# DeepOptimalControl/DeepPicardIteration

Hardware: AMD Instinct MI355X
Metric: SDE-path labels/sec (100-d, 50 Euler steps) per GPU; rel-L2 vs ref (higher is better)
Workload: dtype f32

## Files before the change

deeppicarditeration_amd/_lib.py:

```python
import ctypes
import os
from pathlib import Path

_HERE = Path(__file__).resolve().parent
LIB_PATH = Path(os.environ.get("DPI_HIP_LIB", _HERE / "libdpi_hip.so"))

DPI_ABI_VERSION = 8
DPI_LAUNCH_TIMERS = 256
DPI_OK, DPI_ERR_ARG, DPI_ERR_UNSUPPORTED, DPI_ERR_HIP, DPI_ERR_WORKSPACE = 0, -1, -2, -3, -4
DPI_TAG_T, DPI_TAG_X0, DPI_TAG_X, DPI_TAG_TERM, DPI_TAG_S, DPI_TAG_INT, DPI_TAG_SDGD, DPI_TAG_HTERM, DPI_TAG_HINT = range(1, 10)
DPI_EQ_CHA, DPI_EQ_OU, DPI_EQ_GBM = 1, 2, 3
DPI_ACT_ELU, DPI_ACT_TANH = 1, 2
DPI_HEAD_VALUE, DPI_HEAD_VALUE_GRADIENT, DPI_HEAD_GRADIENT = 0, 1, 2
DPI_TERMINAL, DPI_INTEGRAL, DPI_BOTH = 1, 2, 3
DPI_PREPARED = 4
DPI_PATH_BLOCK = 64
DPI_PATHS_PER_CALL_MAX = 1024 * DPI_PATH_BLOCK
DPI_GEMM_F32, DPI_GEMM_F16X3, DPI_GEMM_AUTO = 0, 1, 2
DPI_STATUS_NONFINITE = 1
DPI_STATUS_HANDOFF = 2
DPI_STATUS_SLOTS = 64
DPI_FAMILY_SPECIALISED, DPI_FAMILY_GENERAL = 0, 1

c_int, c_double, c_float, c_size_t, c_void_p, c_uint32, c_uint64 = (
    ctypes.c_int, ctypes.c_double, ctypes.c_float, ctypes.c_size_t, ctypes.c_void_p, ctypes.c_uint32, ctypes.c_uint64)
P = ctypes.POINTER

SIGNATURES = {
    "dpi_abi_version": (c_int, []),
    "dpi_last_error": (c_int, [ctypes.c_char_p, c_size_t]),
    "dpi_problem_create_cha": (c_int, [c_int, c_double, c_double, c_double, P(c_void_p)]),
    "dpi_problem_create_ou": (c_int, [c_int, c_double, c_double, c_double, c_double, c_double, c_int,
                                      P(c_double), P(c_double), P(c_double), P(c_void_p)]),
    "dpi_problem_create_gbm": (c_int, [c_int, c_double, c_double, c_int, P(c_double), P(c_double), P(c_void_p)]),
    "dpi_problem_set_hessian_approximation": (c_int, [c_void_p, c_int]),
    "dpi_problem_set_estimate_delta_t": (c_int, [c_void_p, c_double]),
    "dpi_problem_destroy": (c_int, [c_void_p]),
    "dpi_net_create_zero": (c_int, [P(c_void_p)]),
    "dpi_net_create_mlp": (c_int, [c_int, c_int, P(c_int), c_int, P(c_float), c_size_t, P(c_void_p)]),
    "dpi_net_create_mlp_head": (c_int, [c_int, c_int, P(c_int), c_int, c_int, P(c_float), c_size_t, P(c_void_p)]),
    "dpi_net_create_mlp_terminal": (c_int, [c_int, c_int, P(c_int), c_int, c_int, c_double, P(c_float), c_size_t,
                                            P(c_void_p)]),
    "dpi_net_create_pisgrad": (c_int, [c_int, c_int, P(c_int), c_double, P(c_float), c_size_t, P(c_void_p)]),
    "dpi_net_destroy": (c_int, [c_void_p]),
    "dpi_pair_family": (c_int, [c_void_p, c_void_p, c_int, P(c_int)]),
    "dpi_general_slots": (c_int, [c_void_p, P(c_int)]),
    "dpi_set_gemm_precision": (c_int, [c_int]),
    "dpi_net_set_precision": (c_int, [c_void_p, c_int]),
    "dpi_net_status": (c_int, [c_void_p, c_int, c_void_p, P(c_int)]),
# ... 100 lines not shown
```

deeppicarditeration_amd/csrc/dpi_device.h:

```cpp
#pragma once
#include <hip/hip_runtime.h>
#include <stdint.h>

#include <cmath>
#include <cstdio>
#include <cstring>
#include <cstdlib>
#include <type_traits>
#include <algorithm>
#include <string>
#include <vector>

#include "../../include/dpi.h"
#include "dpi_eq.h"
#include "dpi_rng.h"

namespace dpi {

typedef float floatx4 __attribute__((ext_vector_type(4)));

constexpr int P = DPI_PATH_BLOCK;
constexpr int NTH = 256;
constexpr int SS = P + 4;
constexpr int WST = 136;
#ifndef DPI_NOISE_UNROLL_FO
#define DPI_NOISE_UNROLL_FO 4
#endif
#ifndef DPI_NOISE_UNROLL_GBM
#define DPI_NOISE_UNROLL_GBM 8
#endif
#ifndef DPI_GBM_WAGPR
#define DPI_GBM_WAGPR 1
#endif
#ifndef DPI_WV_UNIFORM_GBM
#define DPI_WV_UNIFORM_GBM 0
#endif
#ifndef DPI_NOISE_UNROLL_HESS
#define DPI_NOISE_UNROLL_HESS 4
#endif
#ifndef DPI_NOISE_TABLE_FO
#define DPI_NOISE_TABLE_FO 1
#endif
constexpr int NXP_MAX = 128;
constexpr int NXW_MAX = 256;
constexpr int HBS = NXW_MAX;
constexpr int HMAX = 128;

struct NetDev {
  int kind;
  int H, L, nxp;
  int act;
  const float* W1x;
  const float* w1t;
  const float* b1;
  const float* c1;
  const float* W1xT;
  const float* W[4];
  const float* WT[4];
  const float* b[4];
  const float* wout;
  float bout;
  int nxp32;
  const uint32_t* W1xS;
  const uint32_t* W1xTS;
  const uint32_t* WS[4];
  const uint32_t* WTS[4];
  const uint32_t* WU[4];
  float wus[4];
  float hsa[4], hsc[4], hzs[4], hbs[4];
};

__device__ __forceinline__ floatx4 mfma4(float a, float b, floatx4 c) {
  return __builtin_amdgcn_mfma_f32_16x16x4f32(a, b, c, 0, 0, 0);
}
// ... 1512 lines not shown
    for (int g = 0; g < 16; ++g) a += udp[g][tid];
    hb[(size_t)i * HBS + c0 + tid] = c0 + tid < nx ? a : 0.f;
  }
  if (NXW > NXP_MAX) __syncthreads();
  }
  if (tid == 0) fb[i] = Cb;
}

}
#include "dpi_general.h"
namespace dpi {

struct PathArgs {
  const float* tx;
  const float* gx;
  const float* fb;
  const float* bx;
  const float* hb;
  float* partial;
  int n, nbp, m_begin, m_end, K, flags;
  uint32_t k0, k1, c3t, c3s, c3i, c3q, point_base;
  int order;
  int split;
  float* hpart;
  uint32_t c3h1, c3h2;
  float td_dt;
  int* tickets;
  float* rd_moments;
  float* rd_y;
  int* rd_status;
  float rd_invM, rd_bound;
  int rd_add_g;
  const float* noise;
};

struct FusedBase {
  int nbase;
  float* rec;
  unsigned long long* ready;
  uint32_t ready_seq;
  SampleSpec smp;
};

__device__ __forceinline__ unsigned long long ready_word(uint32_t seq) {
  return ((unsigned long long)seq << 32) | (unsigned long long)(~seq);
}
__device__ __forceinline__ void base_publish(const FusedBase& fb, int i) {
  asm volatile("s_waitcnt vmcnt(0)" ::: "memory");
  __syncthreads();
  if (threadIdx.x == 0) {
    __builtin_amdgcn_fence(__ATOMIC_RELEASE, "agent");
    asm volatile("s_waitcnt vmcnt(0)" ::: "memory");
    __hip_atomic_store(fb.ready + i, ready_word(fb.ready_seq), __ATOMIC_RELAXED, __HIP_MEMORY_SCOPE_AGENT);
  }
}
constexpr int BASE_SPIN_MAX = 1 << 20;
__device__ __forceinline__ int& base_ok() {
  __shared__ int ok;
  return ok;
}
__device__ __forceinline__ void base_poll(const FusedBase& fb, const PathArgs& a, int i) {
  if (threadIdx.x == 0) {
    const unsigned long long want = ready_word(fb.ready_seq);
    int it = 0;
    while (__hip_atomic_load(fb.ready + i, __ATOMIC_RELAXED, __HIP_MEMORY_SCOPE_AGENT) != want &&
           ++it < BASE_SPIN_MAX)
      __builtin_amdgcn_s_sleep(8);
// ... 485 lines not shown
      }
    }
  };
  auto integral_rollout = [&]() {
#pragma unroll
    for (int c = 0; c < NBW; ++c) {
      const int j = (3 - wv) + 4 * c;
      if (j < nb) {
        float s0 = 0.f, s1 = 0.f, s2 = 0.f, s3 = 0.f;
        if (INTG && !PRE) {
          noise_sums<NOISE_UNROLL, NOISE_FORM>(a.K, nb, j, m, ig, a.c3i, a.k0, a.k1, s0, s1, s2, s3, ntab);
        }
        float sv[4] = {s0 * BM_SCALE, s1 * BM_SCALE, s2 * BM_SCALE, s3 * BM_SCALE};
        if (INTG && PRE) {
          const float* np = a.noise + ((size_t)(i * a.nbp + blk) * 2 + 1) * (4 * nb) * P + lane;
#pragma unroll
          for (int q = 0; q < 4; ++q) sv[q] = np[(4 * j + q) * P];
        }
#pragma unroll
        for (int q = 0; q < 4; ++q) {
          const int d = 4 * j + q;
          sh.S[d * SS + lane] = d < nx ? sv[q] : 0.f;
          if constexpr (GBM) {
            if (d < nx) {
#pragma unroll
              for (int c = 0; c < NSG; ++c)
                if (c < e.nodes) fst[c] = fmaf(e.gw[c * F + 1 + d], sv[q], fst[c]);
            }
          }
        }
      }
    }
  };
  auto terminal_finish = [&]() -> float {
#pragma unroll
    for (int c = 0; c < NSG; ++c) sh.gst[(wv * P + lane) * NSG + c] = gst[c];
    if constexpr (GBM) {
#pragma unroll
      for (int c = 0; c < NSG; ++c) sh.fst[(wv * P + lane) * NSG + c] = fst[c];
    }
    __syncthreads();
    float gT = 0.f;
    if (TERM) {
#pragma unroll
      for (int c = 0; c < NSG; ++c)
        gst[c] = ((sh.gst[(0 * P + lane) * NSG + c] + sh.gst[(1 * P + lane) * NSG + c]) +
                  sh.gst[(2 * P + lane) * NSG + c]) + sh.gst[(3 * P + lane) * NSG + c];
      gT = Eq<KIND>::gfin(e, gst);
    }
    return TERM ? gT - g_x : 0.f;
  };

  auto integrand = [&]() {
    if constexpr (!GBM) {
      float u = 0.f, gs = 0.f, gA = 0.f, gB = 0.f;
      if (!ZERO && INTG) {
        if constexpr (GEN)
          mlp_tile_gen<KIND, H, ACT, NET, TERMA>(e, net, sh, stash, u, gs, gA, gB);
        else if constexpr (SPLIT)
          mlp_tile_split<KIND, H, L, ACT>(e, net, sh, u, gs, gA, gB);
        else
          mlp_tile<KIND, H, L, ACT>(e, net, sh, nxp / 16, u, gs, gA, gB, nullptr, 0, P);
      }
      const int pp = 16 * wv + (lane & 15);
      if ((lane >> 4) == 0) sh.bsh[pp] = INTG ? tmt * (Eq<KIND>::ffv(e, u, gs, gA, gB) - f_b) : 0.f;
    } else {
      const int jj = lane & 15, qq = lane >> 4, pp = 16 * wv + jj;
      float s1 = 0.f, s2 = 0.f;
      if constexpr (!ZERO) {
        if (INTG) {
          if constexpr (SPLIT)
            mlp_hdiag_split<H, L, ACT>(e, net, sh, nxp / 16, s1, s2);
          else
            mlp_hdiag<H, L, ACT>(e, net, sh, nxp / 16, s1, s2);
        }
      }
      const float vv = (float)(e.sdgd_v > 0 ? e.sdgd_v : nx);
      const float c1 = 0.5f * (1.0f - e.alpha) * (float)nx / vv, c2 = 0.25f * (float)nx / vv;
      float arg[NSG], sn[NSG];
      const float spp = sh.tau[pp], cpp = sh.cmul[pp];
#pragma unroll
      for (int c = 0; c < NSG; ++c) {
        arg[c] = 0.f;
        if (c < e.nodes) {
          const float ws = ((sh.fst[(0 * P + pp) * NSG + c] + sh.fst[(1 * P + pp) * NSG + c]) +
                            sh.fst[(2 * P + pp) * NSG + c]) + sh.fst[(3 * P + pp) * NSG + c];
          arg[c] = fmaf(e.gw[c * F], spp, fmaf(cpp, ws, sh.wx[c]));
        }
        sn[c] = __sinf(arg[c]);
      }
      const float ah = qsum(Eq<KIND>::abs_hess_partial(e, sn, qq, 4));
      float b1 = 0.f, b2 = 0.f;
      for (int d = qq; d < nx; d += 4) {
        const float c = (float)sh.cnt[d * P + pp], h = sh.hb[d];
        b1 = fmaf(c, h, b1);
        b2 = fmaf(c, fabsf(h), b2);
      }
      b1 = qsum(b1);
      b2 = qsum(b2);
      const float f = c1 * s1 + c2 * s2 + Eq<KIND>::exact_scalar_terms(e, arg) - 0.25f * ah;
      const float fbp = f_b + c1 * b1 + c2 * b2;
      if (qq == 0) {
        sh.bsh[pp] = INTG ? tmt * (f - fbp) : 0.f;
        sh.fbp[pp] = fbp;
      }
    }
  };

  bool tlast = false;
  if constexpr (TD) {
    tlast = false;
  } else if constexpr (GEN) {
    tlast = true;
  } else if constexpr (SPLIT && !GBM) {
    tlast = true;
  } else if constexpr (!GBM) {
    if (a.order == 1) tlast = (__builtin_amdgcn_s_getreg((3 << 11) | (16 << 6) | 4) & 1) != 0;
    else if (a.order == 2) tlast = (bid & 1) != 0;
    else if (a.order == 3) tlast = ((bid >> 8) & 1) != 0;
    else if (a.order == 4) tlast = true;
  }
  [[maybe_unused]] auto terminal_value_td = [&]() -> float {
#pragma unroll
    for (int c = 0; c < NBW; ++c) {
      const int j = wv + 4 * c;
      if (j < nb)
#pragma unroll
        for (int q = 0; q < 4; ++q) {
          const int d = 4 * j + q;
          sh.S[d * SS + lane] = d < nx ? ST[c][q] : 0.f;
        }
    }
    if (wv == 0) {
      sh.tau[lane] = t + a.td_dt;
      sh.cmul[lane] = cT;
    }
    __syncthreads();
    float u = 0.f;
    if constexpr (!ZERO) {
      if constexpr (GBM) {
        u = mlp_value_res<H, L, ACT>(net, sh, nxp / 16);
      } else if constexpr (!GEN) {
        float gs, gA, gB;
        if constexpr (SPLIT)
          mlp_tile_split<KIND, H, L, ACT>(e, net, sh, u, gs, gA, gB);
        else
          mlp_tile<KIND, H, L, ACT>(e, net, sh, nxp / 16, u, gs, gA, gB, nullptr, 0, P);
      }
    }
    const int pp = 16 * wv + (lane & 15);
    if ((lane >> 4) == 0) sh.bsh[pp] = u;
    __syncthreads();
    const float uT = sh.bsh[lane];
    if (wv == 0) {
      sh.tau[lane] = s;
      sh.cmul[lane] = cI;
    }
    return uT;
  };
  auto base_poll_ = [&]() {
    if constexpr (FBC) base_poll(fb, a, i);
  };
  auto base_load = [&]() {
    if constexpr (FBC) {
      const bool ok = base_ok() != 0;
      const float* r = fb.rec + (size_t)i * BREC;
      g_x = uniform_f(ok ? rec_load(r) : __builtin_nanf(""));
      f_b = uniform_f(ok ? rec_load(r + 1) : __builtin_nanf(""));
      if (!ZERO) {
        for (int h = tid; h < H; h += NTH) sh.vec[h] = r[32 + h];
        __syncthreads();
      }
    }
  };
  float ap;
  if constexpr (TD) {
    terminal_rollout();
    float uT = 0.f;
    if (td_u && TERM) uT = terminal_value_td();
    integral_rollout();
    ap = terminal_finish();
    if (td_u) ap = TERM ? uT - g_x : 0.f;
    integrand();
    __syncthreads();
  } else if (!tlast) {
    terminal_rollout();
    integral_rollout();
    if constexpr (FBC) {
      base_poll_();
      __syncthreads();
      base_load();
    }
    ap = terminal_finish();
    integrand();
    __syncthreads();
  } else {
    integral_rollout();
    base_poll_();
    __syncthreads();
    base_load();
    integrand();
    terminal_rollout();
    ap = terminal_finish();
  }

  constexpr bool MASK_SCALAR = KIND == DPI_EQ_OU && H == 128 && L == 4 && SPLIT && !TD && NXW == NXP_MAX;
  const bool live = MASK_SCALAR ? lane < a.m_end - a.m_begin - P * blk : m < (uint32_t)a.m_end;
  ap = live ? ap : 0.f;
  const float bp = sh.bsh[lane];
  float* out = a.partial + ((size_t)i * a.nbp + blk) * slab_row(F);
  const float aY = ap * yT, bY = live ? bp * yI : 0.f;
  if constexpr (NXW == NXP_MAX) {
    float col[64];
  #pragma unroll
    for (int c = 0; c < 64; ++c) col[c] = 0.f;
  #pragma unroll
    for (int c = 0; c < 7; ++c) {
// ... 56 lines not shown
          for (int q = 0; q < 4; ++q) {
            const int d = 4 * j + q;
            const float v = d < nx ? fmaf(aY, ST[g0 + c < NBW ? g0 + c : 0][q], bY * sh.S[d * SS + lane]) : 0.f;
            col[8 * c + 2 * q] = v;
            col[8 * c + 2 * q + 1] = v * v;
          }
        }
      }
      if (g0 == 0 && wv == 0) {
        float fbt;
        if constexpr (GBM)
          fbt = sh.fbp[lane];
        else
          fbt = f_b + Eq<KIND>::ffc(e);
        const float c0 = ap + (live ? bp : 0.f) + (INTG ? (live ? fbt : 0.f) * tmt : 0.f);
        col[56] = c0;
        col[57] = c0 * c0;
      }
      const float tot = column_sums64(col);
      const int c = lane >> 3, q = (lane >> 1) & 3, sq = lane & 1;
      const int j = wv + 4 * (g0 + c), d = 4 * j + q;
      if (lane < 56) {
        if (g0 + c < NBW && j < nb && d < nx) out[sq * F + 1 + d] = tot;
      } else if (g0 == 0 && wv == 0 && lane < 58) {
        out[sq * F] = tot;
      }
    }
  }
  if constexpr (HESS) {
    hess_block<KIND, H, L, ZERO, SPLIT, ACT>(e, net, a, sh, i, blk, ig, m, s, smt, tmt, g_x, nxp);
  } else {
    if (a.tickets) fused_reduce(a, i, F, FB ? fb.rec : nullptr);
  }
}

template <int KIND, int H, int L, bool ZERO, bool SPLIT, bool HESS = false, bool TD = false, int ACT = DPI_ACT_ELU,
          int NXW = NXP_MAX>
__global__ __launch_bounds__(256, (k_paths_wgs<KIND, H, L, SPLIT, TD, NXW>())) void k_paths(EqDev e, NetDev net, PathArgs a) {
  paths_body<KIND, H, L, ZERO, SPLIT, HESS, TD, ACT, false, NXW>(e, net, a, FusedBase{});
}
template <int KIND, int H, int L, bool ZERO, bool SPLIT, int ACT = DPI_ACT_ELU>
__global__ __launch_bounds__(256, (k_paths_wgs<KIND, H, L, SPLIT, false>())) void k_paths_fb(EqDev e, NetDev net,
                                                                                            PathArgs a, FusedBase fb) {
  paths_body<KIND, H, L, ZERO, SPLIT, false, false, ACT, true>(e, net, a, fb);
}
template <int KIND, int HCAP, int ACT>
__global__ __launch_bounds__(256, (gen_wgs(HCAP))) void k_paths_gen(EqDev e, NetGen net, PathArgs a, floatx4* stash,
                                                                  unsigned block0) {
  floatx4* const slot = stash + (size_t)blockIdx.x * (gen_slot_floats(net.L, net.ht) / 4);
  paths_body<KIND, HCAP, GEN_LMAX, false, false, false, false, ACT, false, NXP_MAX, NetGen>(e, net, a, FusedBase{},
                                                                                             block0 + blockIdx.x, slot);
}
template <int KIND, int HCAP, int ACT>
__global__ __launch_bounds__(256, (gen_wgs(HCAP))) void k_paths_head(EqDev e, NetGenHead net, PathArgs a) {
  paths_body<KIND, HCAP, GEN_LMAX, false, false, false, false, ACT, false, NXP_MAX, NetGenHead>(e, net, a, FusedBase{},
                                                                                                 blockIdx.x, nullptr);
}
template <int KIND, int HCAP, int ACT>
__global__ __launch_bounds__(256, (gen_wgs(HCAP))) void k_paths_term(EqDev e, NetGen net, PathArgs a, floatx4* stash,
                                                                   unsigned block0) {
  floatx4* const slot = stash + (size_t)blockIdx.x * (gen_slot_floats(net.L, net.ht) / 4);
  paths_body<KIND, HCAP, GEN_LMAX, false, false, false, false, ACT, false, NXP_MAX, NetGen, true>(
      e, net, a, FusedBase{}, block0 + blockIdx.x, slot);
}
template <int KIND, int HCAP, int ACT>
__global__ __launch_bounds__(256, (gen_wgs(HCAP))) void k_paths_head_term(EqDev e, NetGenHead net, PathArgs a) {
// ... 6 lines not shown
```

deeppicarditeration_amd/csrc/dpi_kernels.hip:

```cpp
#include <hip/hip_runtime.h>
#include <stdint.h>

#include <climits>
#include <cmath>
#include <cstdio>
#include <cstring>
#include <cstdlib>
#include <type_traits>
#include <algorithm>
#include <atomic>
#include <mutex>
#include <string>
#include <unordered_map>
#include <vector>

#include "../../include/dpi.h"
#include "dpi_eq.h"
#include "dpi_rng.h"

#include "dpi_dispatch.h"
#include "dpi_pisnet.h"

namespace dpi {

// ... 1258 lines not shown
  L.INP = x3 ? (PIS_CH + pd.nx + 31) & ~31 : r4(PIS_CH + pd.nx);
  o += L.INP;
  L.H0 = o;
  o += PIS_CH;
  L.H1 = o;
  o += PIS_CH;
  for (int l = 0; l < 4; ++l) {
    L.A[l] = o;
    o += l < pd.L ? rw(pd.h[l]) : 0;
  }
  L.NO = o;
  o += rw(pd.nx);
  L.D0 = o;
  o += rw(hmax);
  L.D1 = o;
  o += rw(hmax);
  L.GX = o;
  o += rw(pd.nx);
  L.SS = o;
  o += rw(pd.nx);
  L.ST = o;
  o += rw(pd.nx);
  L.SC = o;
  o += rw(PIS_GST + PIS_PARTS * NSG);
  L.stride = o;
  return L;
}
static int pis_chunk_wg() {
  static const int x = env_int("DPI_PIS_CHUNK", 4096);
  return x >= 1 ? x : 4096;
}

struct WsLayout {
  size_t gx, fb, bx, hb, tk, rec, ready, rows, partial, rq, noise, nq, stash, total;
  int rows_cap;
};
static size_t al256(size_t x) { return (x + 255) & ~size_t(255); }
static bool gbm_noise_prep(dpi_problem p, dpi_net net) {
  static const bool on = env_int("DPI_GBM_PREP", 1) != 0;
  return on && p && net && net->d.kind == 1 && p->e.kind == DPI_EQ_GBM;
}
static WsLayout ws_layout(dpi_net net, int n, int M, int F, bool noise = false) {
  WsLayout w;
  const int H = (net && net->d.kind == 1) ? std::max(net->spec ? net->d.H : 0, net->gen ? net->g.H : 0) : 0;
  const size_t nbp = (size_t)(M + P - 1) / P;
  w.gx = 0;
  w.fb = al256((size_t)n * 4);
  w.bx = w.fb + al256((size_t)n * 4);
  w.hb = w.bx + al256((size_t)n * H * 4);
  w.tk = w.hb + al256((size_t)n * HBS * 4);
  w.rec = w.tk + al256((size_t)n * 4);
  w.ready = w.rec + al256((size_t)n * BREC * 4);
  w.rows = w.ready + al256((size_t)n * 8);
  w.rows_cap = 0;
  size_t rows_bytes = 0;
  if (net && net->d.kind == 2) {
    w.rows_cap = (int)std::min((size_t)n * nbp * P, (size_t)pis_chunk_wg() * P) + n;
    const int stride = std::max(pis_rows_layout(net->pis, false).stride, pis_rows_layout(net->pis, true).stride);
    rows_bytes = al256((size_t)w.rows_cap * stride * 4);
  }
  w.partial = w.rows + rows_bytes;
  w.rq = w.partial + al256((size_t)n * nbp * slab_row(F) * 4);
  w.noise = w.rq + ((net && net->d.kind == 2) ? 256 + (size_t)PIS_CLAIM_SLOTS * 4 : 0);
  const size_t nb4 = (size_t)((F - 1 + 3) / 4) * 4;
  w.nq = w.noise + (noise ? al256((size_t)n * nbp * 2 * nb4 * P * 4) : 0);
  w.total = w.nq + (noise ? 256 + (size_t)PIS_CLAIM_SLOTS * 4 : 0);
  w.stash = w.total;
  if (net && net->d.kind == 1 && net->gen && !net->head) {
    w.stash = al256(w.total);
    w.total = w.stash + al256((size_t)gen_slots(net->g.H) * gen_slot_floats(net->g.L, net->g.ht) * 4);
  }
  return w;
}

static int g_gemm_mode = -1;
static int gemm_mode() {
  if (g_gemm_mode < 0) {
    const char* e = std::getenv("DPI_GEMM");
    g_gemm_mode = !e ? DPI_GEMM_AUTO : std::strcmp(e, "f16x3") == 0 ? DPI_GEMM_F16X3
                                   : std::strcmp(e, "f32") == 0   ? DPI_GEMM_F32
                                                                  : DPI_GEMM_AUTO;
  }
  return g_gemm_mode;
}
static int net_mode(dpi_net net) { return (net && net->precision >= 0) ? net->precision : gemm_mode(); }
static bool mlp_split(dpi_net net) { return net_mode(net) != DPI_GEMM_F32; }
static bool pis_x3(dpi_net net) { return net_mode(net) != DPI_GEMM_F32; }
static int* net_status(dpi_net net) {
  return (net && net->finite && net->status) ? net->status + (size_t)net->slot * STATUS_STRIDE : nullptr;
}

extern "C" int dpi_set_gemm_precision(int mode) {
  if (mode != DPI_GEMM_F32 && mode != DPI_GEMM_F16X3 && mode != DPI_GEMM_AUTO)
    return fail(DPI_ERR_ARG, "gemm precision: 0 = fp32, 1 = fp16-split, 2 = auto");
  g_gemm_mode = mode;
  return 0;
}

template <class F>
static void with_epi(int epi, F f) {
  if (epi == EPI_BIAS)
    f(std::integral_constant<int, EPI_BIAS>{});
  else if (epi == EPI_BIAS_ELU)
// ... 142 lines not shown
  gemm(EPI_BIAS_ELU, R, C, 2 * C, rows + L.E, ld, pd.te0, 2 * C, rows + L.T1, ld, pd.te0b, nullptr, 0, st);
  gemm(EPI_BIAS, R, C, C, rows + L.T1, ld, pd.te2, C, rows + L.IN, ld, pd.te2b, nullptr, 0, st);
  int hs = L.H0, ho = L.H1;
  gemm(EPI_BIAS_ELU, R, C, 2 * C, rows + L.E, ld, pd.sn0, 2 * C, rows + hs, ld, pd.sn0b, nullptr, 0, st);
  for (int j = 0; j < pd.nsm; ++j) {
    gemm(EPI_BIAS_ELU, R, C, C, rows + hs, ld, pd.sn[j], C, rows + ho, ld, pd.snb[j], nullptr, 0, st);
    std::swap(hs, ho);
  }
  int in = C + nx;
  const float* a = rows + L.IN;
  for (int l = 0; l < pd.L; ++l) {
    gemm(EPI_BIAS_ELU, R, pd.h[l], in, a, ld, pd.nn[l], in, rows + L.A[l], ld, pd.nnb[l], nullptr, 0, st);
    a = rows + L.A[l];
    in = pd.h[l];
  }
  gemm(EPI_BIAS, R, nx, in, a, ld, pd.nn[pd.L], in, rows + L.NO, ld, pd.nnb[pd.L], nullptr, 0, st);
  L.H0 = hs;
  if (!vjp) return L;
  int dcur = L.D0, dnext = L.D1;
  gemm(EPI_DELU, R, pd.h[pd.L - 1], nx, rows + L.IN + PIS_IN_OFF, ld, pd.nnT[pd.L], nx, rows + dcur, ld, nullptr,
       rows + L.A[pd.L - 1], ld, st);
  for (int l = pd.L - 1; l >= 1; --l) {
    gemm(EPI_DELU, R, pd.h[l - 1], pd.h[l], rows + dcur, ld, pd.nnT[l], pd.h[l], rows + dnext, ld, nullptr,
         rows + L.A[l - 1], ld, st);
    std::swap(dcur, dnext);
  }
  gemm(EPI_BIAS, R, nx, pd.h[0], rows + dcur, ld, pd.nnT[0], pd.h[0], rows + L.GX, ld, nullptr, nullptr, 0, st);
  L.H0 = hs;
  return L;
}

extern "C" size_t dpi_workspace_bytes(dpi_problem p, dpi_net net, int n, int M) {
  if (!p || n < 0 || M < 0) return 0;
  return ws_layout(net, n, M, 1 + p->e.nx).total;
}
extern "C" size_t dpi_workspace_bytes_prepared(dpi_problem p, dpi_net net, int n, int M) {
  if (!p || n < 0 || M < 0) return 0;
  return ws_layout(net, n, M, 1 + p->e.nx, gbm_noise_prep(p, net)).total;
}

static SampleSpec sample_spec(dpi_problem p, uint64_t seed, uint32_t epoch, uint32_t point_base, float eps,
                              int t_factors, float* tx) {
  SampleSpec s;
  s.tx = tx;
  s.k0 = (uint32_t)seed;
  s.k1 = (uint32_t)(seed >> 32);
  s.c3t = DPI_TAG_T | (epoch << 8);
  s.c3x0 = DPI_TAG_X0 | (epoch << 8);
  s.c3x = DPI_TAG_X | (epoch << 8);
  s.point_base = point_base;
  s.eps = eps;
  s.alpha_init_sqrt = p->alpha_init_sqrt;
  s.t_factors = t_factors;
  return s;
}

extern "C" int dpi_sample_points(dpi_problem p, int n, uint64_t seed, uint32_t epoch, uint32_t point_base, float eps,
                      float* tx, void* stream) {
  return dpi_sample_points_t(p, n, seed, epoch, point_base, eps, 0, tx, stream);
}

extern "C" int dpi_sample_points_t(dpi_problem p, int n, uint64_t seed, uint32_t epoch, uint32_t point_base, float eps,
                                   int t_factors, float* tx, void* stream) {
  if (!p || (!tx && n) || n < 0 || epoch > 0xFFFFFFu || t_factors < 0 || t_factors > 4096)
    return fail(DPI_ERR_ARG, "sample_points: bad arguments (t_factors in [0, 4096])");
  if (n == 0) return 0;
  const int nb = (p->e.nx + 3) >> 2;
  const int total = n * nb;
  const SampleSpec s = sample_spec(p, seed, epoch, point_base, eps, t_factors, tx);
  dim3 grid((total + 255) / 256), block(256);
  hipStream_t st = (hipStream_t)stream;
  switch (p->e.kind) {
    case DPI_EQ_CHA:
      hipLaunchKernelGGL(k_sample_points<DPI_EQ_CHA>, grid, block, 0, st, p->e, n, s);
      break;
    case DPI_EQ_OU:
      hipLaunchKernelGGL(k_sample_points<DPI_EQ_OU>, grid, block, 0, st, p->e, n, s);
      break;
    case DPI_EQ_GBM:
      hipLaunchKernelGGL(k_sample_points<DPI_EQ_GBM>, grid, block, 0, st, p->e, n, s);
      break;
    default:
      return fail(DPI_ERR_UNSUPPORTED, "sample_points: equation kind");
  }
  HIPCHK(hipGetLastError());
  return 0;
}

static bool runs_general(const dpi_problem_s* p, const dpi_net_s* net) {
  return net->d.kind == 1 && net->gen && !(net->spec && spec_shape(p->e.kind, net->d.H, net->d.L));
}
static int general_refusal(const dpi_problem_s* p, const dpi_net_s* net, bool td, bool hess) {
  if (net->term) {
    const char* pre = "a terminal-enforcing network (PicardSolutionEnforceTerminal) runs the general MLP family, which ";
    if (p->e.kind == DPI_EQ_GBM)
      return fail(DPI_ERR_UNSUPPORTED, std::string(pre) + "serves Cha and OU problems only: GBM has no terminal-enforcing "
                                                          "instance");
    if (hess) return fail(DPI_ERR_UNSUPPORTED, std::string(pre) + "has no Hessian labels");
    if (p->e.nx > NXP_MAX)
      return fail(DPI_ERR_UNSUPPORTED, std::string(pre) + "is compiled for nx <= 128 (NXP_MAX)");
    if (td)
      return fail(DPI_ERR_UNSUPPORTED, std::string(pre) + "has no TD estimators (ESTIMATE_DELTA_T > 0)");
    return 0;
  }
  if (net->head) {
    const char* pre = "a ValueGradient / OnlyGradient network (a gradient head) runs the general MLP family, which ";
    if (p->e.kind == DPI_EQ_GBM)
      return fail(DPI_ERR_UNSUPPORTED, std::string(pre) + "serves Cha and OU problems only: GBM needs the Hessian of u, "
                                                          "which a gradient head does not give");
    if (hess) return fail(DPI_ERR_UNSUPPORTED, std::string(pre) + "has no Hessian labels");
    if (p->e.nx > NXP_MAX)
      return fail(DPI_ERR_UNSUPPORTED, std::string(pre) + "is compiled for nx <= 128 (NXP_MAX)");
    if (td)
      return fail(DPI_ERR_UNSUPPORTED, std::string(pre) + "has no TD estimators (ESTIMATE_DELTA_T > 0)");
    return 0;
  }
  const char* pre = "this network has no specialised kernel instance and the general MLP family (up to 8 hidden "
                    "layers of width 256) ";
  if (p->e.kind == DPI_EQ_GBM)
    return fail(DPI_ERR_UNSUPPORTED, std::string(pre) + "serves Cha and OU problems only: GBM nets need one of its compiled "
                                                        "shapes (widths <= 64, at most 3 hidden layers)");
  if (hess) return fail(DPI_ERR_UNSUPPORTED, std::string(pre) + "has no Hessian labels");
  if (p->e.nx > NXP_MAX)
// ... 228 lines not shown
  return 0;
}

static bool fused_reduce_on() { return env_int("DPI_FUSED_REDUCE", 1) != 0; }

static int path_order() { return env_int("DPI_ORDER", 0); }

static size_t hess_extra(int n, int M, int nx, size_t* moff);
static int label_args(dpi_problem p, dpi_net net, const float* tx, int n, int M, int K, uint64_t seed,
                      uint32_t epoch, uint32_t point_base, int m_begin, int m_end, int flags, bool need_moments,
                      const float* moments, void* ws, size_t ws_bytes, WsLayout* w, PathArgs* pa, bool hess = false) {
  const bool prepared = !need_moments || (flags & DPI_PREPARED);
  int rc = check_pair(p, net);
  if (rc) return rc;
  if (hess && runs_general(p, net)) return general_refusal(p, net, false, true);
  if (hess && p->e.kind != DPI_EQ_GBM)
    return fail(DPI_ERR_UNSUPPORTED, "Hessian labels need a SimpleDiffusionEquationWithHessian (GBMEquationComplexExact)");
  if (hess && net->d.kind == 2) return fail(DPI_ERR_UNSUPPORTED, "Hessian labels: MLP or ZeroSolution networks only");
  if (n < 0 || (n && (!tx || !ws || (need_moments && !moments))) || K < 1 || M < 1 || m_begin < 0 || m_end > M ||
      m_end <= m_begin || (m_begin % P) || ((m_end % P) && m_end != M) || !(flags & DPI_BOTH) ||
      (flags & ~(DPI_BOTH | DPI_PREPARED)) || epoch > 0xFFFFFFu)
    return fail(DPI_ERR_ARG,
                hess ? "Hessian labels: bad arguments (m range within [0, M], m_begin a multiple of 64, m_end a "
                       "multiple of 64 or M; K >= 1, flags in DPI_TERMINAL | DPI_INTEGRAL | DPI_PREPARED)"
                     : "label_moments: bad arguments (m range within [0, M], m_begin a multiple of 64, m_end a "
                       "multiple of 64 or M; K >= 1)");
  if (n == 0) return 0;
  const int F = 1 + p->e.nx;
  const int nbp = (m_end - m_begin + P - 1) / P;
  if (nbp > DPI_PATHS_PER_CALL_MAX / P)
    return fail(DPI_ERR_ARG, std::string(hess ? "Hessian labels" : "label_moments") +
                                 ": at most DPI_PATHS_PER_CALL_MAX paths per call");
  const bool noise = prepared && gbm_noise_prep(p, net);
  *w = ws_layout(net, n, M, F, noise);
  if (hess) {
    size_t moff;
    if (ws_bytes < al256(w->total) + hess_extra(n, M, p->e.nx, &moff))
      return fail(DPI_ERR_WORKSPACE, noise ? "workspace too small (dpi_workspace_bytes_hessians_prepared)"
                                           : "workspace too small (dpi_workspace_bytes_hessians)");
  } else if (ws_bytes < w->total)
    return fail(DPI_ERR_WORKSPACE, prepared ? "workspace too small (prepared calls: dpi_workspace_bytes_prepared)"
                                            : "workspace too small");
  char* b = (char*)ws;
  PathArgs& a = *pa;
  std::memset(&a, 0, sizeof(a));
  a.tx = tx;
  a.gx = (const float*)(b + w->gx);
  a.fb = (const float*)(b + w->fb);
  a.bx = (const float*)(b + w->bx);
  a.hb = (const float*)(b + w->hb);
  a.partial = (float*)(b + w->partial);
  a.n = n;
  a.nbp = nbp;
  a.m_begin = m_begin;
  a.m_end = m_end;
  a.K = K;
  a.flags = flags & DPI_BOTH;
  a.k0 = (uint32_t)seed;
  a.k1 = (uint32_t)(seed >> 32);
  a.c3t = DPI_TAG_TERM | (epoch << 8);
  a.c3s = DPI_TAG_S | (epoch << 8);
  a.c3i = DPI_TAG_INT | (epoch << 8);
  a.c3q = DPI_TAG_SDGD | (epoch << 8);
  a.point_base = point_base;
  a.order = path_order();
  a.split = mlp_split(net) ? 1 : 0;
  a.td_dt = p->td_dt;
  return 0;
}

static void arm_fused_reduce(PathArgs& a, dpi_net net, void* ws, const WsLayout& w, int M, int flags, float* moments,
                             float* y, float bound) {
  a.tickets = (int*)((char*)ws + w.tk);
  a.rd_moments = moments;
  a.rd_y = y;
  a.rd_status = net_status(net);
  a.rd_invM = 1.0f / (float)M;
  a.rd_bound = bound;
  a.rd_add_g = (flags & DPI_TERMINAL) ? 1 : 0;
}

static bool stages_prepare(dpi_problem p, dpi_net net);
static int moments_impl(dpi_problem p, dpi_net net, const float* tx, int n, int M, int K, uint64_t seed,
                        uint32_t epoch, uint32_t point_base, int m_begin, int m_end, int flags, float* moments,
                        void* ws, size_t ws_bytes, void* stream, float* y, float bound) {
  WsLayout w;
  PathArgs a;
  int rc = label_args(p, net, tx, n, M, K, seed, epoch, point_base, m_begin, m_end, flags, true, moments, ws, ws_bytes,
                      &w, &a);
  if (rc || n == 0) return rc;
  const int F = 1 + p->e.nx, nbp = a.nbp;
  char* b = (char*)ws;
  float* partial = a.partial;
  hipStream_t st = (hipStream_t)stream;
  if (net->d.kind == 2) {
    if ((rc = pis_paths(p, net, tx, n, K, a, w, b, st, (flags & DPI_PREPARED) != 0))) return rc;
  } else {
    Launch q = path_launch(a, n * nbp, st);
    route_launch(q, p, net, ws, w);
// ... 18 lines not shown
  }
  HIPCHK(hipGetLastError());
  hipLaunchKernelGGL(k_reduce, dim3(n, (2 * F + 3) / 4), dim3(256), 0, st, partial, n, F, nbp, moments,
                     (const float*)(b + w.gx), 1.0f / (float)M, (flags & DPI_TERMINAL) ? 1 : 0, bound, y, F,
                     net_status(net));
  HIPCHK(hipGetLastError());
  return 0;
}

static bool fused_base_on() { return env_int("DPI_FUSED_BASE", 1) != 0; }
static bool fused_base_ok(dpi_problem p, dpi_net net) {
  if (p->td_dt > 0.f || p->e.nx > NXP_MAX || runs_general(p, net)) return false;
  if (net->d.kind == 0) return fused_base_shape(p->e.kind, 0, 0, true, DPI_ACT_ELU);
  return net->d.kind == 1 && mlp_split(net) && fused_base_shape(p->e.kind, net->d.H, net->d.L, false, net->d.act);
}
static std::atomic<uint32_t> g_ready_seq{0};
static uint32_t next_ready_seq() {
  uint32_t s;
  do s = g_ready_seq.fetch_add(1, std::memory_order_relaxed) + 1u;
  while (s == 0u);
  return s;
}

int dpi_sample_with_gradients(dpi_problem p, dpi_net net, int n, int M, int K, uint64_t seed, uint32_t epoch,
                              uint32_t point_base, float eps, int t_factors, int flags, float sample_bound, float* tx,
                              float* y, float* moments, void* ws, size_t ws_bytes, void* stream) {
  int rc = check_pair(p, net);
  if (rc) return rc;
  if (n < 0 || M < 1 || K < 1 || epoch > 0xFFFFFFu || t_factors < 0 || t_factors > 4096)
    return fail(DPI_ERR_ARG, "sample_with_gradients: bad arguments (n >= 0, M, K >= 1, t_factors in [0, 4096])");
  if (n == 0) return 0;
  if (!tx || !y || !moments) return fail(DPI_ERR_ARG, "sample_with_gradients: null tx, y or moments");
  const int F = 1 + p->e.nx;
  const WsLayout w = ws_layout(net, n, M, F);
  if (!ws || ws_bytes < w.total) return fail(DPI_ERR_WORKSPACE, "workspace too small");
  if (net->d.kind == 2) {
    if ((rc = dpi_sample_points_t(p, n, seed, epoch, point_base, eps, t_factors, tx, stream))) return rc;
    return dpi_generate_with_gradients(p, net, tx, n, M, K, seed, epoch, point_base, flags, sample_bound, y, moments, ws,
                                       ws_bytes, stream);
  }
  if (fused_base_ok(p, net) && (M + P - 1) / P <= 64 && fused_reduce_on() && fused_base_on()) {
    WsLayout wl;
    PathArgs a;
    if ((rc = label_args(p, net, tx, n, M, K, seed, epoch, point_base, 0, M, flags, true, moments, ws, ws_bytes, &wl,
                         &a)))
      return rc;
    char* b = (char*)ws;
    arm_fused_reduce(a, net, ws, wl, M, flags, moments, y, sample_bound);
    FusedBase fb{};
    fb.nbase = n;
    fb.rec = (float*)(b + wl.rec);
    fb.ready = (unsigned long long*)(b + wl.ready);
    fb.ready_seq = next_ready_seq();
    fb.smp = sample_spec(p, seed, epoch, point_base, eps, t_factors, tx);
    Launch q = path_launch(a, n + n * a.nbp, (hipStream_t)stream);
    q.fbase = &fb;
    take_timer(q.t0, q.t1);
    if (!dispatch_any(p, net, q))
      return fail(DPI_ERR_UNSUPPORTED, "sample_with_gradients: unsupported equation/network shape");
    HIPCHK(hipGetLastError());
    base_tag_set(ws, n);
    return 0;
  }
  if ((rc = dpi_sample_points_baseline(p, net, n, seed, epoch, point_base, eps, t_factors, tx, ws, ws_bytes, stream)))
    return rc;
  return moments_impl(p, net, tx, n, M, K, seed, epoch, point_base, 0, M, flags, moments, ws, ws_bytes, stream, y,
                      sample_bound);
// ... 143 lines not shown
  return 0;
}

int dpi_sums_reduce(const float* parts, int n_parts, size_t len, float* out, void* stream) {
  if (!parts || !out || n_parts < 1 || n_parts > 1024 || len > 0x7fffffffu)
    return fail(DPI_ERR_ARG, "sums_reduce: bad arguments (1 <= n_parts <= 1024)");
  if (len == 0) return 0;
  hipLaunchKernelGGL(k_reduce_parts, dim3((unsigned)((len + 3) / 4)), dim3(256), 0, (hipStream_t)stream, parts,
                     n_parts, (int)len, out);
  HIPCHK(hipGetLastError());
  return 0;
}

int dpi_label_finalize(dpi_problem p, const float* moments, int n, int M, int flags, float sample_bound, float* y,
                       const void* ws, size_t ws_bytes, void* stream) {
  if (!p || n < 0 || (n && (!moments || !y || !ws)) || M < 1 || ws_bytes < (size_t)n * 4)
    return fail(DPI_ERR_ARG, "label_finalize: bad arguments");
  if (n == 0) return 0;
  const int F = 1 + p->e.nx;
  hipLaunchKernelGGL(k_finalize, dim3((n * F + 255) / 256), dim3(256), 0, (hipStream_t)stream, moments,
                     (const float*)ws, n, F, 1.0f / (float)M, (flags & DPI_TERMINAL) ? 1 : 0, sample_bound, y);
  HIPCHK(hipGetLastError());
  return 0;
}

int dpi_generate_with_gradients(dpi_problem p, dpi_net net, const float* tx, int n, int M, int K, uint64_t seed,
                                uint32_t epoch, uint32_t point_base, int flags, float sample_bound, float* y,
                                float* moments, void* ws, size_t ws_bytes, void* stream) {
  int rc = check_pair(p, net);
  if (rc) return rc;
  if (n < 0 || M < 1 || K < 1) return fail(DPI_ERR_ARG, "generate_with_gradients: bad arguments (n >= 0, M, K >= 1)");
  if (n == 0) return 0;
  const int F = 1 + p->e.nx;
  const WsLayout w = ws_layout(net, n, M, F);
  if (!ws || ws_bytes < w.total) return fail(DPI_ERR_WORKSPACE, "workspace too small");
  if (!moments) return fail(DPI_ERR_ARG, "generate_with_gradients: moments buffer (n*2*(1+nx) floats) required");
  if ((rc = dpi_point_baseline(p, net, tx, n, ws, ws_bytes, stream))) return rc;
  if (!y) return fail(DPI_ERR_ARG, "generate_with_gradients: null y");
  return moments_impl(p, net, tx, n, M, K, seed, epoch, point_base, 0, M, flags, moments, ws, ws_bytes, stream, y,
                      sample_bound);
}

static int hess_tiles(int nx) {
  const int NT = (nx + 15) / 16;
  return NT * (NT + 1) / 2;
}
static size_t hess_extra(int n, int M, int nx, size_t* moff) {
  const int nbp = (M + P - 1) / P;
  *moff = al256((size_t)n * nbp * hess_tiles(nx) * 256 * 4);
  return *moff + al256((size_t)n * 2 * (1 + nx) * 4);
}

size_t dpi_workspace_bytes_hessians(dpi_problem p, dpi_net net, int n, int M) {
  if (!p || n < 0 || M < 0) return 0;
  size_t moff;
  return al256(ws_layout(net, n, M, 1 + p->e.nx).total) + hess_extra(n, M, p->e.nx, &moff);
}
size_t dpi_workspace_bytes_hessians_prepared(dpi_problem p, dpi_net net, int n, int M) {
  if (!p || n < 0 || M < 0) return 0;
  size_t moff;
  return al256(ws_layout(net, n, M, 1 + p->e.nx, gbm_noise_prep(p, net)).total) + hess_extra(n, M, p->e.nx, &moff);
}

static int hess_moments_impl(dpi_problem p, dpi_net net, const float* tx, int n, int M, int K, uint64_t seed,
                             uint32_t epoch, uint32_t point_base, int m_begin, int m_end, int flags, float* moments,
                             float* hsum, void* ws, size_t ws_bytes, void* stream, float* y, float bound) {
  WsLayout w;
// ... 80 lines not shown
```

include/dpi.h:

```cpp
#ifndef DPI_H_
#define DPI_H_

#include <stddef.h>
#include <stdint.h>

#ifdef __cplusplus
extern "C" {
#endif

#define DPI_ABI_VERSION 8

#define DPI_OK 0
#define DPI_ERR_ARG (-1)
#define DPI_ERR_UNSUPPORTED (-2)
#define DPI_ERR_HIP (-3)
#define DPI_ERR_WORKSPACE (-4)

#define DPI_TAG_T 1
#define DPI_TAG_X0 2
#define DPI_TAG_X 3
#define DPI_TAG_TERM 4
#define DPI_TAG_S 5
#define DPI_TAG_INT 6
#define DPI_TAG_SDGD 7
// ... 39 lines not shown
#define DPI_HEAD_GRADIENT 2
int dpi_net_create_mlp_head(int n_in, int n_hidden, const int* widths, int act, int head, const float* params,
                            size_t n_params, dpi_net* out);
int dpi_net_create_mlp_terminal(int n_in, int n_hidden, const int* widths, int act, int head, double T,
                                const float* params, size_t n_params, dpi_net* out);
#define DPI_FAMILY_SPECIALISED 0
#define DPI_FAMILY_GENERAL 1
int dpi_pair_family(dpi_problem p, dpi_net net, int td, int* family);
int dpi_general_slots(dpi_net net, int* slots);
int dpi_net_create_pisgrad(int nx, int n_hidden, const int* hidden, double T, const float* params,
                           size_t n_params, dpi_net* out);
int dpi_net_destroy(dpi_net net);

#define DPI_GEMM_F32 0
#define DPI_GEMM_F16X3 1
#define DPI_GEMM_AUTO 2
int dpi_set_gemm_precision(int mode);

int dpi_net_set_precision(dpi_net net, int mode);

#define DPI_STATUS_NONFINITE 1
#define DPI_STATUS_HANDOFF 2
#define DPI_STATUS_SLOTS 64
int dpi_net_status(dpi_net net, int clear, void* stream, int* status);
int dpi_net_status_slot(dpi_net net, int slot, int clear);
int dpi_net_status_peek(dpi_net net, int slot, int* status);

int dpi_build_id(char* buf, size_t len);

#define DPI_LAUNCH_TIMERS 256
int dpi_launch_timer_arm(int slot);
int dpi_launch_timer_ms(int slot, float* ms);

size_t dpi_workspace_bytes(dpi_problem p, dpi_net net, int n, int M);

size_t dpi_workspace_bytes_prepared(dpi_problem p, dpi_net net, int n, int M);

int dpi_sample_points(dpi_problem p, int n, uint64_t seed, uint32_t epoch, uint32_t point_base, float eps,
                      float* tx, void* stream);

int dpi_sample_points_t(dpi_problem p, int n, uint64_t seed, uint32_t epoch, uint32_t point_base, float eps,
                        int t_factors, float* tx, void* stream);

int dpi_point_baseline(dpi_problem p, dpi_net net, const float* tx, int n, void* ws, size_t ws_bytes,
                       void* stream);

int dpi_label_moments(dpi_problem p, dpi_net net, const float* tx, int n, int M, int K, uint64_t seed,
                      uint32_t epoch, uint32_t point_base, int m_begin, int m_end, int flags, float* moments,
                      void* ws, size_t ws_bytes, void* stream);

int dpi_label_prepare(dpi_problem p, dpi_net net, const float* tx, int n, int M, int K, uint64_t seed,
                      uint32_t epoch, uint32_t point_base, int m_begin, int m_end, int flags, void* ws,
                      size_t ws_bytes, void* stream);

int dpi_label_moments_finalize(dpi_problem p, dpi_net net, const float* tx, int n, int M, int K, uint64_t seed,
                               uint32_t epoch, uint32_t point_base, int flags, float sample_bound, float* y,
                               float* moments, void* ws, size_t ws_bytes, void* stream);

int dpi_moments_reduce(float* parts, int n_parts, int n, int nx, float* out, void* stream);

int dpi_label_finalize(dpi_problem p, const float* moments, int n, int M, int flags, float sample_bound,
                       float* y, const void* ws, size_t ws_bytes, void* stream);

int dpi_generate_with_gradients(dpi_problem p, dpi_net net, const float* tx, int n, int M, int K,
                                uint64_t seed, uint32_t epoch, uint32_t point_base, int flags,
                                float sample_bound, float* y, float* moments, void* ws, size_t ws_bytes,
// ... 31 lines not shown
```

Measured before the change: 185.4 million.

## Park terminal-rollout state in workspace to reorder split fused label phases

In the split, non-GBM fused label kernel, half of the blocks (chosen by a hardware or block-id parity selector) now run the terminal rollout before the baseline poll. They park their terminal state rows in a new global workspace region and publish the terminal sums, then reload the parked rows after the integrand. The other blocks keep the terminal rollout last. The intent is to hide the wait on the baseline poll behind useful terminal work and to stagger phases across blocks. This costs extra global-memory traffic and a larger workspace. Optional s_memtime phase stamps are added behind a compile flag for profiling.

```diff
diff --git a/deeppicarditeration_amd/_lib.py b/deeppicarditeration_amd/_lib.py
--- a/deeppicarditeration_amd/_lib.py
+++ b/deeppicarditeration_amd/_lib.py
@@ -15,6 +15,7 @@
 DPI_TERMINAL, DPI_INTEGRAL, DPI_BOTH = 1, 2, 3
 DPI_PREPARED = 4
 DPI_PATH_BLOCK = 64
+DPI_PARK_MAX_BLOCKS = 2048
 DPI_PATHS_PER_CALL_MAX = 1024 * DPI_PATH_BLOCK
 DPI_GEMM_F32, DPI_GEMM_F16X3, DPI_GEMM_AUTO = 0, 1, 2
 DPI_STATUS_NONFINITE = 1
diff --git a/deeppicarditeration_amd/csrc/dpi_device.h b/deeppicarditeration_amd/csrc/dpi_device.h
--- a/deeppicarditeration_amd/csrc/dpi_device.h
+++ b/deeppicarditeration_amd/csrc/dpi_device.h
@@ -40,6 +40,9 @@
 #endif
 #ifndef DPI_NOISE_TABLE_FO
 #define DPI_NOISE_TABLE_FO 1
+#endif
+#ifndef DPI_PHASE_STAMPS
+#define DPI_PHASE_STAMPS 0
 #endif
 constexpr int NXP_MAX = 128;
 constexpr int NXW_MAX = 256;
@@ -1618,7 +1621,9 @@
   float rd_invM, rd_bound;
   int rd_add_g;
   const float* noise;
+  float* park;
 };
+constexpr int PARK_ROW = 4 * (NXP_MAX / 16) * 64 * 4;
 
 struct FusedBase {
   int nbase;
@@ -2170,13 +2175,15 @@
       }
     }
   };
-  auto terminal_finish = [&]() -> float {
+  auto terminal_publish = [&]() {
 #pragma unroll
     for (int c = 0; c < NSG; ++c) sh.gst[(wv * P + lane) * NSG + c] = gst[c];
     if constexpr (GBM) {
 #pragma unroll
       for (int c = 0; c < NSG; ++c) sh.fst[(wv * P + lane) * NSG + c] = fst[c];
     }
+  };
+  auto terminal_sum = [&]() -> float {
     __syncthreads();
     float gT = 0.f;
     if (TERM) {
@@ -2187,6 +2194,10 @@
       gT = Eq<KIND>::gfin(e, gst);
     }
     return TERM ? gT - g_x : 0.f;
+  };
+  auto terminal_finish = [&]() -> float {
+    terminal_publish();
+    return terminal_sum();
   };
 
   auto integrand = [&]() {
@@ -2245,6 +2256,8 @@
     }
   };
 
+  constexpr bool PARK_SPILLS = NOISE_TAB_SPILLS;
+  constexpr bool PARK = SPLIT && !GBM && !TD && !GEN && NXW == NXP_MAX && !PARK_SPILLS;
   bool tlast = false;
   if constexpr (TD) {
     tlast = false;
@@ -2252,6 +2265,14 @@
     tlast = true;
   } else if constexpr (SPLIT && !GBM) {
     tlast = true;
+    if constexpr (PARK) {
+      if (a.park != nullptr) {
+        if (a.order == 1) tlast = (__builtin_amdgcn_s_getreg((3 << 11) | (16 << 6) | 4) & 1) != 0;
+        else if (a.order == 2) tlast = (bid & 1) != 0;
+        else if (a.order == 3) tlast = ((bid >> 8) & 1) != 0;
+        else if (a.order != 4) tlast = false;
+      }
+    }
   } else if constexpr (!GBM) {
     if (a.order == 1) tlast = (__builtin_amdgcn_s_getreg((3 << 11) | (16 << 6) | 4) & 1) != 0;
     else if (a.order == 2) tlast = (bid & 1) != 0;
@@ -2311,6 +2332,51 @@
       }
     }
   };
+  [[maybe_unused]] auto park_row = [&]() -> floatx4* {
+    return reinterpret_cast<floatx4*>(a.park + (size_t)bid * PARK_ROW) + (wv * NBW) * 64 + lane;
+  };
+  [[maybe_unused]] auto park_store = [&]() {
+    floatx4* const prow = park_row();
+#pragma unroll
+    for (int c = 0; c < NBW; ++c)
+      if (TERM && wv + 4 * c < nb) prow[64 * c] = floatx4{ST[c][0], ST[c][1], ST[c][2], ST[c][3]};
+  };
+  [[maybe_unused]] auto park_load = [&]() {
+    const floatx4* const prow = park_row();
+#pragma unroll
+    for (int c = 0; c < NBW; ++c) {
+      floatx4 v = {0.f, 0.f, 0.f, 0.f};
+      if (TERM && wv + 4 * c < nb) v = prow[64 * c];
+      ST[c][0] = v[0];
+      ST[c][1] = v[1];
+      ST[c][2] = v[2];
+      ST[c][3] = v[3];
+    }
+  };
+  [[maybe_unused]] auto stamp = [&](int k) {
+#if DPI_PHASE_STAMPS
+    if constexpr (PARK) {
+      if (a.park != nullptr && nb <= 28) {
+        unsigned long long tk;
+        __builtin_amdgcn_sched_barrier(0);
+        asm volatile("s_memtime %0\n\ts_waitcnt lgkmcnt(0)" : "=s"(tk)::"memory");
+        __builtin_amdgcn_sched_barrier(0);
+        unsigned long long* const sp =
+            reinterpret_cast<unsigned long long*>(a.park + (size_t)bid * PARK_ROW + (NBW - 1) * 64 * 4);
+        if (lane == 0) {
+          sp[4 + 8 * wv + k] = tk;
+          if (k == 0 && wv == 0) {
+            sp[0] = (unsigned long long)__builtin_amdgcn_s_getreg((31 << 11) | 4) |
+                    ((unsigned long long)__builtin_amdgcn_s_getreg((31 << 11) | 20) << 32);
+            sp[1] = tlast ? 1ull : 0ull;
+          }
+        }
+      }
+    }
+#else
+    (void)k;
+#endif
+  };
   float ap;
   if constexpr (TD) {
     terminal_rollout();
@@ -2321,6 +2387,31 @@
     if (td_u) ap = TERM ? uT - g_x : 0.f;
     integrand();
     __syncthreads();
+  } else if constexpr (PARK) {
+    stamp(0);
+    if (!tlast) {
+      terminal_rollout();
+      park_store();
+      terminal_publish();
+      stamp(1);
+    }
+    integral_rollout();
+    stamp(2);
+    base_poll_();
+    __syncthreads();
+    base_load();
+    stamp(3);
+    integrand();
+    stamp(4);
+    if (tlast) {
+      terminal_rollout();
+      terminal_publish();
+    } else {
+      park_load();
+    }
+    stamp(5);
+    ap = terminal_sum();
+    stamp(6);
   } else if (!tlast) {
     terminal_rollout();
     integral_rollout();
@@ -2443,6 +2534,7 @@
   } else {
     if (a.tickets) fused_reduce(a, i, F, FB ? fb.rec : nullptr);
   }
+  stamp(7);
 }
 
 template <int KIND, int H, int L, bool ZERO, bool SPLIT, bool HESS = false, bool TD = false, int ACT = DPI_ACT_ELU,
diff --git a/deeppicarditeration_amd/csrc/dpi_kernels.hip b/deeppicarditeration_amd/csrc/dpi_kernels.hip
--- a/deeppicarditeration_amd/csrc/dpi_kernels.hip
+++ b/deeppicarditeration_amd/csrc/dpi_kernels.hip
@@ -1314,15 +1314,17 @@
 }
 
 struct WsLayout {
-  size_t gx, fb, bx, hb, tk, rec, ready, rows, partial, rq, noise, nq, stash, total;
+  size_t gx, fb, bx, hb, tk, rec, ready, rows, partial, rq, noise, nq, stash, park, total;
   int rows_cap;
+  size_t park_rows;
 };
 static size_t al256(size_t x) { return (x + 255) & ~size_t(255); }
 static bool gbm_noise_prep(dpi_problem p, dpi_net net) {
   static const bool on = env_int("DPI_GBM_PREP", 1) != 0;
   return on && p && net && net->d.kind == 1 && p->e.kind == DPI_EQ_GBM;
 }
-static WsLayout ws_layout(dpi_net net, int n, int M, int F, bool noise = false) {
+static bool park_pair(dpi_problem p, dpi_net net);
+static WsLayout ws_layout(dpi_net net, int n, int M, int F, bool noise = false, bool park = false) {
   WsLayout w;
   const int H = (net && net->d.kind == 1) ? std::max(net->spec ? net->d.H : 0, net->gen ? net->g.H : 0) : 0;
   const size_t nbp = (size_t)(M + P - 1) / P;
@@ -1351,6 +1353,13 @@
   if (net && net->d.kind == 1 && net->gen && !net->head) {
     w.stash = al256(w.total);
     w.total = w.stash + al256((size_t)gen_slots(net->g.H) * gen_slot_floats(net->g.L, net->g.ht) * 4);
+  }
+  w.park = w.total;
+  w.park_rows = 0;
+  if (park) {
+    w.park_rows = (size_t)DPI_PARK_MAX_BLOCKS;
+    w.park = al256(w.total);
+    w.total = w.park + w.park_rows * PARK_ROW * 4;
   }
   return w;
 }
@@ -1559,11 +1568,11 @@
 
 extern "C" size_t dpi_workspace_bytes(dpi_problem p, dpi_net net, int n, int M) {
   if (!p || n < 0 || M < 0) return 0;
-  return ws_layout(net, n, M, 1 + p->e.nx).total;
+  return ws_layout(net, n, M, 1 + p->e.nx, false, park_pair(p, net)).total;
 }
 extern "C" size_t dpi_workspace_bytes_prepared(dpi_problem p, dpi_net net, int n, int M) {
   if (!p || n < 0 || M < 0) return 0;
-  return ws_layout(net, n, M, 1 + p->e.nx, gbm_noise_prep(p, net)).total;
+  return ws_layout(net, n, M, 1 + p->e.nx, gbm_noise_prep(p, net), park_pair(p, net)).total;
 }
 
 static SampleSpec sample_spec(dpi_problem p, uint64_t seed, uint32_t epoch, uint32_t point_base, float eps,
@@ -1616,6 +1625,9 @@
 
 static bool runs_general(const dpi_problem_s* p, const dpi_net_s* net) {
   return net->d.kind == 1 && net->gen && !(net->spec && spec_shape(p->e.kind, net->d.H, net->d.L));
+}
+static bool park_pair(dpi_problem p, dpi_net net) {
+  return p && net && net->d.kind == 1 && p->e.kind != DPI_EQ_GBM && p->e.nx <= NXP_MAX;
 }
 static int general_refusal(const dpi_problem_s* p, const dpi_net_s* net, bool td, bool hess) {
   if (net->term) {
@@ -1910,7 +1922,7 @@
     return fail(DPI_ERR_ARG, std::string(hess ? "Hessian labels" : "label_moments") +
                                  ": at most DPI_PATHS_PER_CALL_MAX paths per call");
   const bool noise = prepared && gbm_noise_prep(p, net);
-  *w = ws_layout(net, n, M, F, noise);
+  *w = ws_layout(net, n, M, F, noise, park_pair(p, net));
   if (hess) {
     size_t moff;
     if (ws_bytes < al256(w->total) + hess_extra(n, M, p->e.nx, &moff))
@@ -1943,6 +1955,8 @@
   a.point_base = point_base;
   a.order = path_order();
   a.split = mlp_split(net) ? 1 : 0;
+  if (a.split && !runs_general(p, net) && w->park_rows && (size_t)n * nbp <= w->park_rows)
+    a.park = (float*)(b + w->park);
   a.td_dt = p->td_dt;
   return 0;
 }
@@ -2027,7 +2041,7 @@
   if (n == 0) return 0;
   if (!tx || !y || !moments) return fail(DPI_ERR_ARG, "sample_with_gradients: null tx, y or moments");
   const int F = 1 + p->e.nx;
-  const WsLayout w = ws_layout(net, n, M, F);
+  const WsLayout w = ws_layout(net, n, M, F, false, park_pair(p, net));
   if (!ws || ws_bytes < w.total) return fail(DPI_ERR_WORKSPACE, "workspace too small");
   if (net->d.kind == 2) {
     if ((rc = dpi_sample_points_t(p, n, seed, epoch, point_base, eps, t_factors, tx, stream))) return rc;
@@ -2237,7 +2251,7 @@
   if (n < 0 || M < 1 || K < 1) return fail(DPI_ERR_ARG, "generate_with_gradients: bad arguments (n >= 0, M, K >= 1)");
   if (n == 0) return 0;
   const int F = 1 + p->e.nx;
-  const WsLayout w = ws_layout(net, n, M, F);
+  const WsLayout w = ws_layout(net, n, M, F, false, park_pair(p, net));
   if (!ws || ws_bytes < w.total) return fail(DPI_ERR_WORKSPACE, "workspace too small");
   if (!moments) return fail(DPI_ERR_ARG, "generate_with_gradients: moments buffer (n*2*(1+nx) floats) required");
   if ((rc = dpi_point_baseline(p, net, tx, n, ws, ws_bytes, stream))) return rc;
diff --git a/include/dpi.h b/include/dpi.h
--- a/include/dpi.h
+++ b/include/dpi.h
@@ -95,6 +95,7 @@
 int dpi_launch_timer_arm(int slot);
 int dpi_launch_timer_ms(int slot, float* ms);
 
+#define DPI_PARK_MAX_BLOCKS 2048
 size_t dpi_workspace_bytes(dpi_problem p, dpi_net net, int n, int M);
 
 size_t dpi_workspace_bytes_prepared(dpi_problem p, dpi_net net, int n, int M);
```

After: 193.3 million (median of 6 runs). 1.04x the previous value.
